# scaomath/galerkin-transformer

Hardware: AMD Instinct MI355X
Metric: training samples/s, Darcy 141x141 Galerkin encoder (fwd+loss+bwd+clip+Adam) (higher is better)
Workload: dtype f32 (operands split into 2 fp16 terms under a running per-row / per-tile power-of-two scale, 3 products on the f16 MFMA pipe, f32 accumulate; fp32-class results: the 1e-5 parity suite passes in this mode; packed-B token GEMMs, convolutions, weight gradients, regression head and the Fourier attention

## Files before the change

galerkin-transformer_amd/csrc/gt_ffn.hip:

```cpp
#include <cstdint>
#include <cstdlib>
#include <algorithm>

#include "gt_common.h"

namespace gt {

typedef __attribute__((address_space(3))) void* ffn_lds_ptr;
typedef const __attribute__((address_space(1))) void* ffn_glb_ptr;

constexpr int FFN_BM = 64, FFN_BK = 16;
constexpr int FFN_STAGE = FFN_BM * FFN_BK * 4;
constexpr int FFN_HSTRIDE = FFN_STAGE + 16;
constexpr int FFN_E0 = 120, FFN_TARGET = 13, FFN_LIMIT = 15;
constexpr int FFN_EP_SW = 36;

__device__ __attribute__((aligned(16))) float ffn_zero[4] = {0.f, 0.f, 0.f, 0.f};

struct FfnP {
    const float* x; const float* res; float* hid; float* out;
    const float* b1; const float* b2;
    const void* Bp1; const void* Bp2;
    int T, d, f;
    int KS1, NT1, KS2, NT2;
    DropDev dh, dout;
    int act;
    uint32_t* bits_out; const uint32_t* bits_in;
    int bwd;
    float e1_scale;
    float* out2; DropDev d2;
};

__device__ __forceinline__ float ffn_alt(int parity) { return (parity & 1) ? -1.f : 1.f; }

__device__ __forceinline__ void ffn_frag(const char* __restrict__ img, int row, int lh, float (&v)[8]) {
    const int s = (row >> 2) & 3;
    const f32x4 a = *reinterpret_cast<const f32x4*>(img + row * 64 + (((2 * lh) ^ s) << 4));
    const f32x4 b = *reinterpret_cast<const f32x4*>(img + row * 64 + (((2 * lh + 1) ^ s) << 4));
    v[0] = a[0]; v[1] = a[1]; v[2] = a[2]; v[3] = a[3];
    v[4] = b[0]; v[5] = b[1]; v[6] = b[2]; v[7] = b[3];
}

template <int NJ>
__device__ __forceinline__ void ffn_tile_stage(const float (&v)[8], int& ea, float sgn, const f16x8 (&bn)[NJ][2],
                                               f32x16 (&acc)[NJ]) {
    float amax = fmaxf(fmaxf(fabsf(v[0]), fabsf(v[1])), fabsf(v[2]));
    amax = fmaxf(fmaxf(amax, fabsf(v[3])), fabsf(v[4]));
    amax = fmaxf(fmaxf(amax, fabsf(v[5])), fabsf(v[6]));
    amax = xor32_max(fmaxf(amax, fabsf(v[7])));
    const int ex = (int)(__float_as_uint(amax) >> 23);
    const bool need = ex + ea - 127 >= FFN_LIMIT;
    if (__any(need)) {
        const int enew = need ? FFN_TARGET + 127 - ex : ea;
        const int dlt = enew - ea;
        const float f = dlt < -126 ? 0.f : pow2_f(dlt);
#pragma unroll
        for (int j = 0; j < NJ; ++j)
#pragma unroll
            for (int e = 0; e < 16; ++e) acc[j][e] *= f;
        ea = enew;
    }
    const float sv = pow2_f(ea) * sgn;
    uint32_t q[4][2];
#pragma unroll
    for (int t = 0; t < 4; ++t) f16_mulsplit_pair(v[2 * t], sv, v[2 * t + 1], sv, q[t][0], q[t][1]);
    f16x8 am[2];
#pragma unroll
    for (int pl = 0; pl < 2; ++pl) am[pl] = __builtin_bit_cast(f16x8, u32x4{q[0][pl], q[1][pl], q[2][pl], q[3][pl]});
#pragma unroll
    for (int s = 1; s >= 0; --s)
#pragma unroll
        for (int pa = 0; pa < 2; ++pa) {
            const int pb = s - pa;
            if (pb < 0 || pb > 1) continue;
#pragma unroll
            for (int j = 0; j < NJ; ++j) acc[j] = __builtin_amdgcn_mfma_f32_32x32x16_f16(bn[j][pb], am[pa], acc[j], 0, 0, 0);
        }
}

__device__ __forceinline__ void ffn_unscale(f32x16& a, int ea, int eb, float sgn) {
    const int et = -(ea + eb), etc = et < -126 ? -126 : (et > 126 ? 126 : et);
    const float sg = pow2_f(etc) * sgn;
#pragma unroll
    for (int e = 0; e < 16; ++e) a[e] *= (e & 1) ? -sg : sg;
    if (et != etc) {
#pragma unroll
        for (int e = 0; e < 16; ++e) a[e] = ldexpf(a[e], et - etc);
    }
}

#define FFN_WAIT_B_(N, bn)                                                                                             \
    asm volatile("s_waitcnt vmcnt(" #N ")" : "+v"(bn[0][0]), "+v"(bn[0][1]), "+v"(bn[1][0]), "+v"(bn[1][1])::"memory")
#define FFN_WAIT_AB_(N, bn)                                                                                            \
    asm volatile("s_waitcnt vmcnt(" #N ")\n\ts_barrier"                                                                \
                 : "+v"(bn[0][0]), "+v"(bn[0][1]), "+v"(bn[1][0]), "+v"(bn[1][1])::"memory")

constexpr int FFN_HST_SW = 68;
constexpr int FFN_PS_TAB = 4 * 64 * FFN_HST_SW * 4;
template <bool PS>
__global__ __launch_bounds__(256, 2) void ffn_fwd16_kernel(const FfnP p) {
    extern __shared__ __attribute__((aligned(16))) char smem[];
    char* const himg = smem;
    const int tid = threadIdx.x, lane = tid & 63, wave = tid >> 6;
    const int lr = lane & 31, lh = lane >> 5;
    int tile;
    {
        const int tiles = gridDim.x, q = tiles >> 3, r = tiles & 7;
        const int x = blockIdx.x & 7, j = blockIdx.x >> 3;
        tile = (x < r ? x * (q + 1) : r * (q + 1) + (x - r) * q) + j;
    }
    const int m0 = tile * FFN_BM;
    const uint32_t voff = lane * 16;

    const int wn_u = __builtin_amdgcn_readfirstlane(wave);
    const char* bbase = reinterpret_cast<const char*>(p.Bp1) + (int64_t)(wn_u * 2) * p.KS1 * 1024;
    const int64_t bplane = (int64_t)p.NT1 * p.KS1 * 1024;
    f16x8 bs0[2][2], bs1[2][2], bs2[2][2];
    auto loadb = [&](int ks, f16x8 (&bn)[2][2]) {
#pragma unroll
        for (int j = 0; j < 2; ++j)
#pragma unroll
            for (int pl = 0; pl < 2; ++pl) {
                const char* sp = bbase + pl * bplane + ((int64_t)j * p.KS1 + ks) * 1024;
                asm volatile("global_load_dwordx4 %0, %1, %2" : "=v"(bn[j][pl]) : "v"(voff), "s"(sp));
            }
    };
    f32x4 b1v[2][4];
#pragma unroll
    for (int j = 0; j < 2; ++j)
#pragma unroll
        for (int g = 0; g < 4; ++g)
            b1v[j][g] = p.b1 ? *reinterpret_cast<const f32x4*>(p.b1 + 64 * wave + 32 * j + 8 * g + 4 * lh) : f32x4{0.f, 0.f, 0.f, 0.f};
    {
        const int row = 16 * wave + (lane >> 2), slot = lane & 3;
        const int g = slot ^ ((row >> 2) & 3);
        const int xr = m0 + row;
        const float* src0 = xr < p.T ? p.x + (int64_t)xr * p.d + 4 * g : ffn_zero;
        const int step = xr < p.T ? FFN_BK : 0;
#pragma unroll
        for (int st = 0; st < 8; ++st)
            __builtin_amdgcn_global_load_lds((ffn_glb_ptr)(src0 + st * step), (ffn_lds_ptr)(himg + st * FFN_HSTRIDE + wave * 1024), 16, 0, 0);
    }
    f32x16 acc[2][2];
#pragma unroll
    for (int i = 0; i < 2; ++i)
#pragma unroll
        for (int j = 0; j < 2; ++j)
#pragma unroll
            for (int e = 0; e < 16; ++e) acc[i][j][e] = 0.f;
    int ea[2] = {FFN_E0, FFN_E0};
    auto stage = [&](int kt, f16x8 (&bn)[2][2]) {
        const char* sa = himg + kt * FFN_HSTRIDE;
#pragma unroll
        for (int i = 0; i < 2; ++i) {
            float v[8];
            ffn_frag(sa, 32 * i + lr, lh, v);
            ffn_tile_stage<2>(v, ea[i], ffn_alt(i), bn, acc[i]);
        }
    };
    loadb(0, bs0); loadb(1, bs1); loadb(2, bs2);
    FFN_WAIT_AB_(8, bs0);
#pragma unroll
    for (int j = 0; j < 2; ++j)
#pragma unroll
        for (int g = 0; g < 4; ++g) asm volatile("" : "+v"(b1v[j][g]));
    stage(0, bs0); loadb(3, bs0);
    FFN_WAIT_B_(8, bs1); stage(1, bs1); loadb(4, bs1);
    FFN_WAIT_B_(8, bs2); stage(2, bs2); loadb(5, bs2);
    FFN_WAIT_B_(8, bs0); stage(3, bs0); loadb(6, bs0);
    FFN_WAIT_B_(8, bs1); stage(4, bs1); loadb(7, bs1);
    FFN_WAIT_B_(8, bs2); stage(5, bs2);
    FFN_WAIT_B_(4, bs0); stage(6, bs0);
    FFN_WAIT_B_(0, bs1); stage(7, bs1);

    const char* bbase2 = reinterpret_cast<const char*>(p.Bp2) + (int64_t)wn_u * p.KS2 * 1024;
    const int64_t bplane2 = (int64_t)p.NT2 * p.KS2 * 1024;
    f16x8 cn0[1][2], cn1[1][2], cn2[1][2], cn3[1][2];
    auto loadb2 = [&](int ks, f16x8 (&bn)[1][2]) {
#pragma unroll
        for (int pl = 0; pl < 2; ++pl) {
            const char* sp = bbase2 + pl * bplane2 + (int64_t)ks * 1024;
            asm volatile("global_load_dwordx4 %0, %1, %2" : "=v"(bn[0][pl]) : "v"(voff), "s"(sp));
        }
    };
    loadb2(0, cn0); loadb2(1, cn1); loadb2(2, cn2); loadb2(3, cn3);
    asm volatile("s_barrier" ::: "memory");

    int er[2] = {0, 0};
    if constexpr (PS) {
        const int* ebp = reinterpret_cast<const int*>(reinterpret_cast<const char*>(p.Bp1) + 2 * bplane) + wn_u * 2;
        const uint32_t key = drop_key_dev(p.dh);
        float* tab = reinterpret_cast<float*>(smem + FFN_PS_TAB);
#pragma unroll
        for (int i = 0; i < 2; ++i) {
            const int row = 32 * i + lr;
            const uint32_t di0 = (uint32_t)((int64_t)(m0 + row) * p.f + 64 * wave + 4 * lh);
            float amax = 0.f;
            const int64_t widx = ((int64_t)(tile * 4 + wave) * 64 + lane) * 2 + i;
            const uint32_t bin = p.bwd ? p.bits_in[widx] : 0u;
            uint32_t bout = 0u;
#pragma unroll
            for (int j = 0; j < 2; ++j) {
                ffn_unscale(acc[i][j], ea[i], ebp[j], ffn_alt(i));
#pragma unroll
                for (int g = 0; g < 4; ++g)
#pragma unroll
                    for (int t = 0; t < 4; ++t) {
                        float y;
                        if (p.bwd) {
                            y = ((bin >> (16 * j + 4 * g + t)) & 1u) ? acc[i][j][4 * g + t] * p.e1_scale : 0.f;
                        } else {
                            y = acc[i][j][4 * g + t] + b1v[j][g][t];
                            if (p.act == GT_ACT_RELU) y = fmaxf(y, 0.f);
                            if (p.dh.thresh) y *= drop_mul(p.dh, key, di0 + 32 * j + 8 * g + t);
                            bout |= (y > 0.f ? 1u : 0u) << (16 * j + 4 * g + t);
                        }
                        acc[i][j][4 * g + t] = y;
                        amax = fmaxf(amax, fabsf(y));
                    }
            }
            if (p.bits_out) p.bits_out[widx] = bout;
            amax = xor32_max(amax);
            if (lh == 0) tab[wave * 64 + row] = amax;
        }
        asm volatile("s_waitcnt lgkmcnt(0)\n\ts_barrier" ::: "memory");
#pragma unroll
        for (int i = 0; i < 2; ++i) {
            const int row = 32 * i + lr;
            const float a = fmaxf(fmaxf(tab[row], tab[64 + row]), fmaxf(tab[128 + row], tab[192 + row]));
            const int ex = (int)(__float_as_uint(a) >> 23);
            er[i] = ex == 0 ? 0 : min(FFN_E0, FFN_TARGET + 127 - ex);
            const float sv = pow2_f(er[i]) * ffn_alt(i);
#pragma unroll
            for (int j = 0; j < 2; ++j)
#pragma unroll
                for (int g = 0; g < 4; ++g) {
                    uint32_t h0, l0, h1, l1;
                    f16_mulsplit_pair(acc[i][j][4 * g], sv, acc[i][j][4 * g + 1], sv, h0, l0);
                    f16_mulsplit_pair(acc[i][j][4 * g + 2], sv, acc[i][j][4 * g + 3], sv, h1, l1);
                    const int st = 4 * wave + 2 * j + (g >> 1);
                    char* dst = smem + (((st * 2 + (g & 1)) * 64 + row) * 16 + lh * 8);
                    *reinterpret_cast<uint2*>(dst) = uint2{h0, h1};
                    *reinterpret_cast<uint2*>(dst + 16 * 64 * 32) = uint2{l0, l1};
                }
        }
    } else {
        const int* ebp = reinterpret_cast<const int*>(reinterpret_cast<const char*>(p.Bp1) + 2 * bplane) + wn_u * 2;
        const uint32_t key = drop_key_dev(p.dh);
#pragma unroll
        for (int i = 0; i < 2; ++i) {
            const int row = 32 * i + lr, swz = (row >> 2) & 3;
            const uint32_t di0 = (uint32_t)((int64_t)(m0 + row) * p.f + 64 * wave + 4 * lh);
#pragma unroll
            for (int j = 0; j < 2; ++j) {
                ffn_unscale(acc[i][j], ea[i], ebp[j], ffn_alt(i));
#pragma unroll
                for (int g = 0; g < 4; ++g) {
                    f32x4 h;
#pragma unroll
                    for (int t = 0; t < 4; ++t) {
                        float y = acc[i][j][4 * g + t] + b1v[j][g][t];
                        if (p.act == GT_ACT_RELU) y = fmaxf(y, 0.f);
                        if (p.dh.thresh) y *= drop_mul(p.dh, key, di0 + 32 * j + 8 * g + t);
                        h[t] = y;
                    }
                    const int st = 4 * wave + 2 * j + (g >> 1), gq = 2 * (g & 1) + lh;
                    *reinterpret_cast<f32x4*>(himg + st * FFN_HSTRIDE + row * 64 + ((gq ^ swz) << 4)) = h;
                }
            }
        }
    }
    asm volatile("s_waitcnt lgkmcnt(0)\n\ts_barrier" ::: "memory");

#define FFN_WAIT_B2_(N, bn) asm volatile("s_waitcnt vmcnt(" #N ")" : "+v"(bn[0][0]), "+v"(bn[0][1])::"memory")
    f32x16 acc2[2][1];
#pragma unroll
    for (int i = 0; i < 2; ++i)
#pragma unroll
        for (int e = 0; e < 16; ++e) acc2[i][0][e] = 0.f;
    int ea2[2] = {FFN_E0, FFN_E0};
    auto stage2 = [&](int kt2, f16x8 (&bn)[1][2]) {
#pragma unroll
        for (int i = 0; i < 2; ++i) {
            if constexpr (PS) {
                const char* fr = smem + (((kt2 * 2 + lh) * 64 + 32 * i + lr) * 16);
                const f16x8 a0 = *reinterpret_cast<const f16x8*>(fr);
                const f16x8 a1 = *reinterpret_cast<const f16x8*>(fr + 16 * 64 * 32);
                acc2[i][0] = __builtin_amdgcn_mfma_f32_32x32x16_f16(bn[0][0], a1, acc2[i][0], 0, 0, 0);
                acc2[i][0] = __builtin_amdgcn_mfma_f32_32x32x16_f16(bn[0][1], a0, acc2[i][0], 0, 0, 0);
                acc2[i][0] = __builtin_amdgcn_mfma_f32_32x32x16_f16(bn[0][0], a0, acc2[i][0], 0, 0, 0);
            } else {
                float v[8];
                ffn_frag(himg + kt2 * FFN_HSTRIDE, 32 * i + lr, lh, v);
                ffn_tile_stage<1>(v, ea2[i], ffn_alt(i), bn, acc2[i]);
            }
        }
    };
    FFN_WAIT_B2_(6, cn0); stage2(0, cn0); loadb2(4, cn0);
    FFN_WAIT_B2_(6, cn1); stage2(1, cn1); loadb2(5, cn1);
    FFN_WAIT_B2_(6, cn2); stage2(2, cn2); loadb2(6, cn2);
    FFN_WAIT_B2_(6, cn3); stage2(3, cn3); loadb2(7, cn3);
    FFN_WAIT_B2_(6, cn0); stage2(4, cn0); loadb2(8, cn0);
    FFN_WAIT_B2_(6, cn1); stage2(5, cn1); loadb2(9, cn1);
    FFN_WAIT_B2_(6, cn2); stage2(6, cn2); loadb2(10, cn2);
    FFN_WAIT_B2_(6, cn3); stage2(7, cn3); loadb2(11, cn3);
    FFN_WAIT_B2_(6, cn0); stage2(8, cn0); loadb2(12, cn0);
    FFN_WAIT_B2_(6, cn1); stage2(9, cn1); loadb2(13, cn1);
    FFN_WAIT_B2_(6, cn2); stage2(10, cn2); loadb2(14, cn2);
    FFN_WAIT_B2_(6, cn3); stage2(11, cn3); loadb2(15, cn3);
    FFN_WAIT_B2_(6, cn0); stage2(12, cn0);
    FFN_WAIT_B2_(4, cn1); stage2(13, cn1);
    FFN_WAIT_B2_(2, cn2); stage2(14, cn2);
    FFN_WAIT_B2_(0, cn3); stage2(15, cn3);
#undef FFN_WAIT_B2_
    {
        const int* ebp2 = reinterpret_cast<const int*>(reinterpret_cast<const char*>(p.Bp2) + 2 * bplane2) + wn_u;
#pragma unroll
        for (int i = 0; i < 2; ++i) ffn_unscale(acc2[i][0], PS ? er[i] : ea2[i], ebp2[0], ffn_alt(i));
    }

    const int c8 = lane & 7, rsub = lane >> 3;
    const int ocol = 32 * wave + 4 * c8;
    f32x4 rs[8];
    if (p.res) {
#pragma unroll
        for (int it = 0; it < 8; ++it) {
            const int m = m0 + 8 * it + rsub;
            rs[it] = m < p.T ? *reinterpret_cast<const f32x4*>(p.res + (int64_t)m * p.d + ocol) : f32x4{0.f, 0.f, 0.f, 0.f};
        }
    }
    const f32x4 b2v = p.b2 ? *reinterpret_cast<const f32x4*>(p.b2 + ocol) : f32x4{0.f, 0.f, 0.f, 0.f};
    if constexpr (PS) {
        asm volatile("s_waitcnt lgkmcnt(0)\n\ts_barrier" ::: "memory");
        float* hs = reinterpret_cast<float*>(smem) + wave * (64 * FFN_HST_SW);
#pragma unroll
        for (int i = 0; i < 2; ++i)
#pragma unroll
            for (int j = 0; j < 2; ++j)
#pragma unroll
                for (int g = 0; g < 4; ++g)
                    *reinterpret_cast<f32x4*>(hs + (32 * i + lr) * FFN_HST_SW + 32 * j + 8 * g + 4 * lh) =
                        f32x4{acc[i][j][4 * g], acc[i][j][4 * g + 1], acc[i][j][4 * g + 2], acc[i][j][4 * g + 3]};
        asm volatile("s_waitcnt lgkmcnt(0)" ::: "memory");
        const int c4 = lane & 15, r4 = lane >> 4;
#pragma unroll 4
        for (int it = 0; it < 16; ++it) {
            const int row = 4 * it + r4;
            const f32x4 h = *reinterpret_cast<const f32x4*>(hs + row * FFN_HST_SW + 4 * c4);
            if (m0 + row < p.T) *reinterpret_cast<f32x4*>(p.hid + (int64_t)(m0 + row) * p.f + 64 * wave + 4 * c4) = h;
        }
        asm volatile("s_waitcnt lgkmcnt(0)" ::: "memory");
    } else {
    {
        const int st = lane >> 2, gq = lane & 3;
#pragma unroll 4
        for (int rr = 0; rr < 16; ++rr) {
            const int row = 16 * wave + rr;
            const f32x4 h = *reinterpret_cast<const f32x4*>(himg + st * FFN_HSTRIDE + row * 64 + ((gq ^ ((row >> 2) & 3)) << 4));
            if (m0 + row < p.T) *reinterpret_cast<f32x4*>(p.hid + (int64_t)(m0 + row) * p.f + 4 * lane) = h;
        }
    }
    asm volatile("s_waitcnt lgkmcnt(0)\n\ts_barrier" ::: "memory");
    }
    {
        float* stg = reinterpret_cast<float*>(smem) + wave * (PS ? 64 * FFN_HST_SW : 64 * FFN_EP_SW);
#pragma unroll
        for (int i = 0; i < 2; ++i)
#pragma unroll
            for (int g = 0; g < 4; ++g)
                *reinterpret_cast<f32x4*>(stg + (32 * i + lr) * FFN_EP_SW + 8 * g + 4 * lh) =
                    f32x4{acc2[i][0][4 * g], acc2[i][0][4 * g + 1], acc2[i][0][4 * g + 2], acc2[i][0][4 * g + 3]};
        asm volatile("s_waitcnt lgkmcnt(0)" ::: "memory");
        const uint32_t key = drop_key_dev(p.dout);
#pragma unroll
        for (int it = 0; it < 8; ++it) {
            const int r = 8 * it + rsub, m = m0 + r;
            f32x4 v = *reinterpret_cast<const f32x4*>(stg + r * FFN_EP_SW + 4 * c8);
            const uint32_t di = (uint32_t)((int64_t)m * p.d + ocol);
#pragma unroll
            for (int t = 0; t < 4; ++t) {
                float y = v[t] + b2v[t];
                if (p.dout.thresh) y *= drop_mul(p.dout, key, di + t);
                v[t] = p.res ? rs[it][t] + y : y;
            }
            if (m < p.T) *reinterpret_cast<f32x4*>(p.out + (int64_t)m * p.d + ocol) = v;
            if (p.out2) {
                const uint32_t key2 = drop_key_dev(p.d2);
                if (p.d2.thresh) {
#pragma unroll
                    for (int t = 0; t < 4; ++t) v[t] *= drop_mul(p.d2, key2, di + t);
                }
                if (m < p.T) *reinterpret_cast<f32x4*>(p.out2 + (int64_t)m * p.d + ocol) = v;
            }
        }
    }
}

}

using namespace gt;

extern "C" int64_t gt_ffn_fwd_ws_bytes(int64_t T, int32_t d, int32_t f) {
    gt_gemm_desc a, b;
    gt_gemm_desc_init(&a); gt_gemm_desc_init(&b);
    a.M = b.M = (int32_t)std::min<int64_t>(T, 1 << 30);
    a.N = f; a.K = d; a.lda = d; a.ldb = d; a.ldc = f; a.precision = GT_PREC_F16X2;
    b.N = d; b.K = f; b.lda = f; b.ldb = f; b.ldc = d; b.precision = GT_PREC_F16X2;
    a.A = a.B = b.A = b.B = reinterpret_cast<const float*>(uintptr_t(16));
    a.C = b.C = reinterpret_cast<float*>(uintptr_t(16));
    const int64_t pa = gt_gemm_packed_b_bytes(&a), pb = gt_gemm_packed_b_bytes(&b);
    return (pa > 0 && pb > 0) ? pa + pb : 0;
}

static int ffn_launch(FfnP& p, const gt_gemm_desc& a, const gt_gemm_desc& b, const void* p1, const void* p2, void* ws,
                      int64_t ws_bytes, void* stream) {
    auto al = [](const void* q) { return (reinterpret_cast<uintptr_t>(q) & 15) == 0; };
    if ((p1 == nullptr) != (p2 == nullptr)) return GT_EINVAL;
    const int64_t pa = gt_gemm_packed_b_bytes(&a), pb = gt_gemm_packed_b_bytes(&b);
    if (pa <= 0 || pb <= 0) return GT_ENOTSUP;
    if (!p1) {
        if (!ws || ws_bytes < pa + pb || !al(ws)) return GT_EWS;
        gt_gemm_desc two[2] = {a, b};
        void* outs[2] = {ws, reinterpret_cast<char*>(ws) + pa};
        if (int rc = gt_gemm_pack_b_many(two, outs, 2, stream)) return rc;
        p1 = outs[0]; p2 = outs[1];
    } else if (!al(p1) || !al(p2)) return GT_EALIGN;
    p.Bp1 = p1; p.Bp2 = p2;
    static const int presplit = [] { const char* e = getenv("GT_FFN_PRESPLIT"); return e ? atoi(e) : 1; }();
    if (!presplit && (p.bwd || p.bits_out)) return GT_ENOTSUP;
    const size_t lds0 = (size_t)16 * FFN_HSTRIDE, lds1 = (size_t)FFN_PS_TAB + 1024;
    const unsigned tiles = (unsigned)(((int64_t)p.T + FFN_BM - 1) / FFN_BM);
    hipStream_t st = (hipStream_t)stream;
    if (presplit) {
        if (int rc = gt_allow_dynamic_lds<ffn_fwd16_kernel<true>>(lds1)) return rc;
        hipLaunchKernelGGL(ffn_fwd16_kernel<true>, dim3(tiles), dim3(256), lds1, st, p);
    } else {
        if (int rc = gt_allow_dynamic_lds<ffn_fwd16_kernel<false>>(lds0)) return rc;
        hipLaunchKernelGGL(ffn_fwd16_kernel<false>, dim3(tiles), dim3(256), lds0, st, p);
    }
    GT_LAUNCH_CHECK();
    return 0;
}

static bool ffn_shape_ok(int64_t T, int32_t d, int32_t f) { return d == 128 && f == 256 && T >= 16384 && T <= (1 << 30); }

extern "C" int64_t gt_ffn_bits_bytes(int64_t T) { return T > 0 ? ((T + FFN_BM - 1) / FFN_BM) * 4 * 64 * 2 * (int64_t)sizeof(uint32_t) : 0; }

extern "C" int gt_ffn_fwd(const float* x, int64_t T, int32_t d, int32_t f, const float* W1, const float* b1,
                          const float* W2, const float* b2, const float* res, const gt_dropout* drop_h,
                          const gt_dropout* drop_o, int32_t act, float* hid, float* out, void* relu_bits,
                          const void* w1_packed, const void* w2_packed, void* ws, int64_t ws_bytes, void* stream) {
    if (!x || !W1 || !W2 || !hid || !out || T <= 0) return GT_EINVAL;
    if (!ffn_shape_ok(T, d, f) || (act != GT_ACT_RELU && act != GT_ACT_NONE)) return GT_ENOTSUP;
    if ((drop_h && drop_h->p > 0.f && !drop_h->seed) || (drop_o && drop_o->p > 0.f && !drop_o->seed)) return GT_EINVAL;
    if ((drop_h && (drop_h->p < 0.f || drop_h->p >= 1.f)) || (drop_o && (drop_o->p < 0.f || drop_o->p >= 1.f))) return GT_EINVAL;
    auto al = [](const void* q) { return (reinterpret_cast<uintptr_t>(q) & 15) == 0; };
    if (!al(x) || !al(W1) || !al(W2) || !al(hid) || !al(out) || !al(res) || !al(b1) || !al(b2) || !al(relu_bits)) return GT_EALIGN;
    gt_gemm_desc a, b;
    gt_gemm_desc_init(&a); gt_gemm_desc_init(&b);
    a.M = b.M = (int32_t)T;
    a.N = f; a.K = d; a.A = x; a.lda = d; a.B = W1; a.ldb = d; a.C = hid; a.ldc = f; a.precision = GT_PREC_F16X2;
    b.N = d; b.K = f; b.A = hid; b.lda = f; b.B = W2; b.ldb = f; b.C = out; b.ldc = d; b.precision = GT_PREC_F16X2;
    FfnP p{x, res, hid, out, b1, b2, nullptr, nullptr, (int)T, d, f,
           d / 16, ((f + 127) / 128) * 4, f / 16, ((d + 127) / 128) * 4, make_drop(drop_h), make_drop(drop_o), act,
           reinterpret_cast<uint32_t*>(relu_bits), nullptr, 0, 1.f, nullptr, make_drop(nullptr)};
    return ffn_launch(p, a, b, w1_packed, w2_packed, ws, ws_bytes, stream);
}

extern "C" int gt_ffn_bwd(const float* gm, int64_t T, int32_t d, int32_t f, const float* W2, const float* W1,
                          const void* relu_bits, float hid_scale, const float* res, float* gh, float* dx, float* dx_masked,
                          const gt_dropout* mask2, const void* w2_packed, const void* w1_packed, void* ws, int64_t ws_bytes,
                          void* stream) {
    if (!gm || !W1 || !W2 || !relu_bits || !gh || !dx || T <= 0) return GT_EINVAL;
    if (!ffn_shape_ok(T, d, f)) return GT_ENOTSUP;
    if (mask2 && (mask2->p < 0.f || mask2->p >= 1.f || (mask2->p > 0.f && !mask2->seed))) return GT_EINVAL;
    auto al = [](const void* q) { return (reinterpret_cast<uintptr_t>(q) & 15) == 0; };
    if (!al(gm) || !al(W1) || !al(W2) || !al(gh) || !al(dx) || !al(res) || !al(dx_masked) || !al(relu_bits)) return GT_EALIGN;
    gt_gemm_desc a, b;
    gt_gemm_desc_init(&a); gt_gemm_desc_init(&b);
    a.M = b.M = (int32_t)T;
    a.N = f; a.K = d; a.A = gm; a.lda = d; a.B = W2; a.ldb = f; a.layout_b = 1; a.C = gh; a.ldc = f; a.precision = GT_PREC_F16X2;
    b.N = d; b.K = f; b.A = gh; b.lda = f; b.B = W1; b.ldb = d; b.layout_b = 1; b.C = dx; b.ldc = d; b.precision = GT_PREC_F16X2;
    FfnP p{gm, res, gh, dx, nullptr, nullptr, nullptr, nullptr, (int)T, d, f,
           d / 16, ((f + 127) / 128) * 4, f / 16, ((d + 127) / 128) * 4, make_drop(nullptr), make_drop(nullptr), GT_ACT_NONE,
           nullptr, reinterpret_cast<const uint32_t*>(relu_bits), 1, hid_scale, dx_masked, make_drop(mask2)};
    return ffn_launch(p, a, b, w2_packed, w1_packed, ws, ws_bytes, stream);
}
```

Before: 6238.

## Make presplit FFN kernel persistent with prefetched next-tile X and residual loads

The presplit FFN forward kernel becomes persistent. The grid is capped at two blocks per CU, and each block loops over a contiguous range of row tiles. The next tile's X rows are prefetched into registers during the epilogue and split into fp16 hi/lo planes in LDS once per tile, instead of being re-split on every MFMA stage. Residual loads, dropout keys and per-column exponent and bias loads are moved earlier or hoisted out of the loop to overlap with compute. This trades higher register pressure and more complex wait counts for less launch/tail overhead and less redundant splitting work.

New measurement: 6214. Within noise of the previous version (-0.4%).

```diff
diff --git a/galerkin-transformer_amd/csrc/gt_ffn.hip b/galerkin-transformer_amd/csrc/gt_ffn.hip
--- a/galerkin-transformer_amd/csrc/gt_ffn.hip
+++ b/galerkin-transformer_amd/csrc/gt_ffn.hip
@@ -97,24 +97,76 @@
 
 constexpr int FFN_HST_SW = 68;
 constexpr int FFN_PS_TAB = 4 * 64 * FFN_HST_SW * 4;
+constexpr int FFN_XPLANE = 8 * 2 * 64 * 16;
 template <bool PS>
 __global__ __launch_bounds__(256, 2) void ffn_fwd16_kernel(const FfnP p) {
     extern __shared__ __attribute__((aligned(16))) char smem[];
     char* const himg = smem;
     const int tid = threadIdx.x, lane = tid & 63, wave = tid >> 6;
     const int lr = lane & 31, lh = lane >> 5;
-    int tile;
+    int tile, tend, tstep;
     {
-        const int tiles = gridDim.x, q = tiles >> 3, r = tiles & 7;
+        const int tiles = (p.T + FFN_BM - 1) / FFN_BM, q = tiles >> 3, r = tiles & 7;
+        const int nb = gridDim.x >> 3, nr = gridDim.x & 7;
         const int x = blockIdx.x & 7, j = blockIdx.x >> 3;
-        tile = (x < r ? x * (q + 1) : r * (q + 1) + (x - r) * q) + j;
-    }
-    const int m0 = tile * FFN_BM;
+        const int t0 = x < r ? x * (q + 1) : r * (q + 1) + (x - r) * q;
+        tile = t0 + j;
+        tend = t0 + (x < r ? q + 1 : q);
+        tstep = nb + (x < nr ? 1 : 0);
+    }
+    if (tile >= tend) return;
     const uint32_t voff = lane * 16;
 
     const int wn_u = __builtin_amdgcn_readfirstlane(wave);
     const char* bbase = reinterpret_cast<const char*>(p.Bp1) + (int64_t)(wn_u * 2) * p.KS1 * 1024;
     const int64_t bplane = (int64_t)p.NT1 * p.KS1 * 1024;
+    const char* bbase2 = reinterpret_cast<const char*>(p.Bp2) + (int64_t)wn_u * p.KS2 * 1024;
+    const int64_t bplane2 = (int64_t)p.NT2 * p.KS2 * 1024;
+    const int xrow = 16 * wave + (lane >> 2), xg = lane & 3;
+    f32x4 xr[8];
+    auto loadx = [&](int t, bool live) {
+        const int r = t * FFN_BM + xrow;
+        const bool in = live && r < p.T;
+        const float* src0 = in ? p.x + (int64_t)r * p.d + 4 * xg : ffn_zero;
+        const int step = in ? FFN_BK : 0;
+#pragma unroll
+        for (int st = 0; st < 8; ++st) asm volatile("global_load_dwordx4 %0, %1, off" : "=v"(xr[st]) : "v"(src0 + st * step));
+    };
+    if constexpr (PS) loadx(tile, true);
+    const uint32_t key_h = drop_key_dev(p.dh);
+    const uint32_t key_o = drop_key_dev(p.dout);
+    const uint32_t key_2 = drop_key_dev(p.d2);
+    const int* ebp = reinterpret_cast<const int*>(reinterpret_cast<const char*>(p.Bp1) + 2 * bplane) + wn_u * 2;
+    const int eb1[2] = {ebp[0], ebp[1]};
+    const int eb2 = (reinterpret_cast<const int*>(reinterpret_cast<const char*>(p.Bp2) + 2 * bplane2))[wn_u];
+    const int c8 = lane & 7, rsub = lane >> 3;
+    const int ocol = 32 * wave + 4 * c8;
+    const f32x4 b2v = p.b2 ? *reinterpret_cast<const f32x4*>(p.b2 + ocol) : f32x4{0.f, 0.f, 0.f, 0.f};
+    if constexpr (PS) {
+        asm volatile("s_waitcnt vmcnt(0)"
+                     : "+v"(xr[0]), "+v"(xr[1]), "+v"(xr[2]), "+v"(xr[3]), "+v"(xr[4]), "+v"(xr[5]), "+v"(xr[6]), "+v"(xr[7])::"memory");
+    }
+
+    for (;;) {
+    const int m0 = tile * FFN_BM;
+    const bool more = tile + tstep < tend;
+    f32x4 rs[8];
+    auto loadres = [&]() {
+#pragma unroll
+        for (int it = 0; it < 8; ++it) {
+            const int m = m0 + 8 * it + rsub;
+            const float* src = (p.res && m < p.T) ? p.res + (int64_t)m * p.d + ocol : ffn_zero;
+            asm volatile("global_load_dwordx4 %0, %1, off" : "=v"(rs[it]) : "v"(src));
+        }
+    };
+    asm volatile("" : "+s"(bbase), "+s"(bbase2));
+    f32x4 b1v[2][4];
+#pragma unroll
+    for (int j = 0; j < 2; ++j)
+#pragma unroll
+        for (int g = 0; g < 4; ++g)
+            b1v[j][g] = p.b1 ? *reinterpret_cast<const f32x4*>(p.b1 + 64 * wave + 32 * j + 8 * g + 4 * lh) : f32x4{0.f, 0.f, 0.f, 0.f};
+
     f16x8 bs0[2][2], bs1[2][2], bs2[2][2];
     auto loadb = [&](int ks, f16x8 (&bn)[2][2]) {
 #pragma unroll
@@ -125,18 +177,12 @@
                 asm volatile("global_load_dwordx4 %0, %1, %2" : "=v"(bn[j][pl]) : "v"(voff), "s"(sp));
             }
     };
-    f32x4 b1v[2][4];
-#pragma unroll
-    for (int j = 0; j < 2; ++j)
-#pragma unroll
-        for (int g = 0; g < 4; ++g)
-            b1v[j][g] = p.b1 ? *reinterpret_cast<const f32x4*>(p.b1 + 64 * wave + 32 * j + 8 * g + 4 * lh) : f32x4{0.f, 0.f, 0.f, 0.f};
-    {
+    if constexpr (!PS) {
         const int row = 16 * wave + (lane >> 2), slot = lane & 3;
         const int g = slot ^ ((row >> 2) & 3);
-        const int xr = m0 + row;
-        const float* src0 = xr < p.T ? p.x + (int64_t)xr * p.d + 4 * g : ffn_zero;
-        const int step = xr < p.T ? FFN_BK : 0;
+        const int xm = m0 + row;
+        const float* src0 = xm < p.T ? p.x + (int64_t)xm * p.d + 4 * g : ffn_zero;
+        const int step = xm < p.T ? FFN_BK : 0;
 #pragma unroll
         for (int st = 0; st < 8; ++st)
             __builtin_amdgcn_global_load_lds((ffn_glb_ptr)(src0 + st * step), (ffn_lds_ptr)(himg + st * FFN_HSTRIDE + wave * 1024), 16, 0, 0);
@@ -149,17 +195,61 @@
 #pragma unroll
             for (int e = 0; e < 16; ++e) acc[i][j][e] = 0.f;
     int ea[2] = {FFN_E0, FFN_E0};
+    uint32_t bin[2] = {0u, 0u};
+    loadb(0, bs0); loadb(1, bs1); loadb(2, bs2);
+    if constexpr (PS) {
+        asm volatile("s_waitcnt lgkmcnt(0)\n\ts_barrier" ::: "memory");
+        {
+            const uint32_t* bsrc = p.bwd ? p.bits_in + ((int64_t)(tile * 4 + wave) * 64 + lane) * 2 : reinterpret_cast<const uint32_t*>(ffn_zero);
+            bin[0] = bsrc[0]; bin[1] = bsrc[1];
+        }
+        float amax = 0.f;
+#pragma unroll
+        for (int st = 0; st < 8; ++st)
+#pragma unroll
+            for (int t = 0; t < 4; ++t) amax = fmaxf(amax, fabsf(xr[st][t]));
+        amax = fmaxf(amax, __shfl_xor(amax, 1));
+        amax = fmaxf(amax, __shfl_xor(amax, 2));
+        const int ex = (int)(__float_as_uint(amax) >> 23);
+        const int ex_row = ex == 0 ? 0 : min(FFN_E0, FFN_TARGET + 127 - ex);
+        const float sv = pow2_f(ex_row) * ffn_alt(xrow >> 5);
+        char* dst = smem + (((xg >> 1) * 64 + xrow) * 16 + (xg & 1) * 8);
+#pragma unroll
+        for (int st = 0; st < 8; ++st) {
+            uint32_t h0, l0, h1, l1;
+            f16_mulsplit_pair(xr[st][0], sv, xr[st][1], sv, h0, l0);
+            f16_mulsplit_pair(xr[st][2], sv, xr[st][3], sv, h1, l1);
+            *reinterpret_cast<uint2*>(dst + st * 2048) = uint2{h0, h1};
+            *reinterpret_cast<uint2*>(dst + st * 2048 + FFN_XPLANE) = uint2{l0, l1};
+        }
+        int* xtab = reinterpret_cast<int*>(smem + FFN_PS_TAB);
+        if (xg == 0) xtab[xrow] = ex_row;
+        asm volatile("s_waitcnt lgkmcnt(0)\n\ts_barrier" ::: "memory");
+#pragma unroll
+        for (int i = 0; i < 2; ++i) ea[i] = xtab[32 * i + lr];
+    }
     auto stage = [&](int kt, f16x8 (&bn)[2][2]) {
-        const char* sa = himg + kt * FFN_HSTRIDE;
 #pragma unroll
         for (int i = 0; i < 2; ++i) {
-            float v[8];
-            ffn_frag(sa, 32 * i + lr, lh, v);
-            ffn_tile_stage<2>(v, ea[i], ffn_alt(i), bn, acc[i]);
+            if constexpr (PS) {
+                const char* fr = smem + (((kt * 2 + lh) * 64 + 32 * i + lr) * 16);
+                const f16x8 a0 = *reinterpret_cast<const f16x8*>(fr);
+                const f16x8 a1 = *reinterpret_cast<const f16x8*>(fr + FFN_XPLANE);
+#pragma unroll
+                for (int j = 0; j < 2; ++j) acc[i][j] = __builtin_amdgcn_mfma_f32_32x32x16_f16(bn[j][1], a0, acc[i][j], 0, 0, 0);
+#pragma unroll
+                for (int j = 0; j < 2; ++j) acc[i][j] = __builtin_amdgcn_mfma_f32_32x32x16_f16(bn[j][0], a1, acc[i][j], 0, 0, 0);
+#pragma unroll
+                for (int j = 0; j < 2; ++j) acc[i][j] = __builtin_amdgcn_mfma_f32_32x32x16_f16(bn[j][0], a0, acc[i][j], 0, 0, 0);
+            } else {
+                float v[8];
+                ffn_frag(himg + kt * FFN_HSTRIDE, 32 * i + lr, lh, v);
+                ffn_tile_stage<2>(v, ea[i], ffn_alt(i), bn, acc[i]);
+            }
         }
     };
-    loadb(0, bs0); loadb(1, bs1); loadb(2, bs2);
-    FFN_WAIT_AB_(8, bs0);
+    if constexpr (PS) FFN_WAIT_B_(8, bs0);
+    else FFN_WAIT_AB_(8, bs0);
 #pragma unroll
     for (int j = 0; j < 2; ++j)
 #pragma unroll
@@ -173,8 +263,7 @@
     FFN_WAIT_B_(4, bs0); stage(6, bs0);
     FFN_WAIT_B_(0, bs1); stage(7, bs1);
 
-    const char* bbase2 = reinterpret_cast<const char*>(p.Bp2) + (int64_t)wn_u * p.KS2 * 1024;
-    const int64_t bplane2 = (int64_t)p.NT2 * p.KS2 * 1024;
+    if constexpr (PS) asm volatile("" : "+v"(bin[0]), "+v"(bin[1]));
     f16x8 cn0[1][2], cn1[1][2], cn2[1][2], cn3[1][2];
     auto loadb2 = [&](int ks, f16x8 (&bn)[1][2]) {
 #pragma unroll
@@ -188,8 +277,6 @@
 
     int er[2] = {0, 0};
     if constexpr (PS) {
-        const int* ebp = reinterpret_cast<const int*>(reinterpret_cast<const char*>(p.Bp1) + 2 * bplane) + wn_u * 2;
-        const uint32_t key = drop_key_dev(p.dh);
         float* tab = reinterpret_cast<float*>(smem + FFN_PS_TAB);
 #pragma unroll
         for (int i = 0; i < 2; ++i) {
@@ -197,22 +284,21 @@
             const uint32_t di0 = (uint32_t)((int64_t)(m0 + row) * p.f + 64 * wave + 4 * lh);
             float amax = 0.f;
             const int64_t widx = ((int64_t)(tile * 4 + wave) * 64 + lane) * 2 + i;
-            const uint32_t bin = p.bwd ? p.bits_in[widx] : 0u;
             uint32_t bout = 0u;
 #pragma unroll
             for (int j = 0; j < 2; ++j) {
-                ffn_unscale(acc[i][j], ea[i], ebp[j], ffn_alt(i));
+                ffn_unscale(acc[i][j], ea[i], eb1[j], ffn_alt(i));
 #pragma unroll
                 for (int g = 0; g < 4; ++g)
 #pragma unroll
                     for (int t = 0; t < 4; ++t) {
                         float y;
                         if (p.bwd) {
-                            y = ((bin >> (16 * j + 4 * g + t)) & 1u) ? acc[i][j][4 * g + t] * p.e1_scale : 0.f;
+                            y = ((bin[i] >> (16 * j + 4 * g + t)) & 1u) ? acc[i][j][4 * g + t] * p.e1_scale : 0.f;
                         } else {
                             y = acc[i][j][4 * g + t] + b1v[j][g][t];
                             if (p.act == GT_ACT_RELU) y = fmaxf(y, 0.f);
-                            if (p.dh.thresh) y *= drop_mul(p.dh, key, di0 + 32 * j + 8 * g + t);
+                            if (p.dh.thresh) y *= drop_mul(p.dh, key_h, di0 + 32 * j + 8 * g + t);
                             bout |= (y > 0.f ? 1u : 0u) << (16 * j + 4 * g + t);
                         }
                         acc[i][j][4 * g + t] = y;
@@ -224,6 +310,7 @@
             if (lh == 0) tab[wave * 64 + row] = amax;
         }
         asm volatile("s_waitcnt lgkmcnt(0)\n\ts_barrier" ::: "memory");
+        loadx(tile + tstep, more);
 #pragma unroll
         for (int i = 0; i < 2; ++i) {
             const int row = 32 * i + lr;
@@ -245,15 +332,13 @@
                 }
         }
     } else {
-        const int* ebp = reinterpret_cast<const int*>(reinterpret_cast<const char*>(p.Bp1) + 2 * bplane) + wn_u * 2;
-        const uint32_t key = drop_key_dev(p.dh);
 #pragma unroll
         for (int i = 0; i < 2; ++i) {
             const int row = 32 * i + lr, swz = (row >> 2) & 3;
             const uint32_t di0 = (uint32_t)((int64_t)(m0 + row) * p.f + 64 * wave + 4 * lh);
 #pragma unroll
             for (int j = 0; j < 2; ++j) {
-                ffn_unscale(acc[i][j], ea[i], ebp[j], ffn_alt(i));
+                ffn_unscale(acc[i][j], ea[i], eb1[j], ffn_alt(i));
 #pragma unroll
                 for (int g = 0; g < 4; ++g) {
                     f32x4 h;
@@ -261,7 +346,7 @@
                     for (int t = 0; t < 4; ++t) {
                         float y = acc[i][j][4 * g + t] + b1v[j][g][t];
                         if (p.act == GT_ACT_RELU) y = fmaxf(y, 0.f);
-                        if (p.dh.thresh) y *= drop_mul(p.dh, key, di0 + 32 * j + 8 * g + t);
+                        if (p.dh.thresh) y *= drop_mul(p.dh, key_h, di0 + 32 * j + 8 * g + t);
                         h[t] = y;
                     }
                     const int st = 4 * wave + 2 * j + (g >> 1), gq = 2 * (g & 1) + lh;
@@ -296,40 +381,36 @@
             }
         }
     };
-    FFN_WAIT_B2_(6, cn0); stage2(0, cn0); loadb2(4, cn0);
-    FFN_WAIT_B2_(6, cn1); stage2(1, cn1); loadb2(5, cn1);
-    FFN_WAIT_B2_(6, cn2); stage2(2, cn2); loadb2(6, cn2);
-    FFN_WAIT_B2_(6, cn3); stage2(3, cn3); loadb2(7, cn3);
+#define FFN_WAIT_B2X_(bn)                                                                                              \
+    do {                                                                                                               \
+        if constexpr (PS) FFN_WAIT_B2_(14, bn);                                                                        \
+        else FFN_WAIT_B2_(6, bn);                                                                                      \
+    } while (0)
+    FFN_WAIT_B2X_(cn0); stage2(0, cn0); loadb2(4, cn0);
+    FFN_WAIT_B2X_(cn1); stage2(1, cn1); loadb2(5, cn1);
+    FFN_WAIT_B2X_(cn2); stage2(2, cn2); loadb2(6, cn2);
+    FFN_WAIT_B2X_(cn3); stage2(3, cn3); loadb2(7, cn3);
+#undef FFN_WAIT_B2X_
     FFN_WAIT_B2_(6, cn0); stage2(4, cn0); loadb2(8, cn0);
+    if constexpr (PS)
+        asm volatile("" : "+v"(xr[0]), "+v"(xr[1]), "+v"(xr[2]), "+v"(xr[3]), "+v"(xr[4]), "+v"(xr[5]), "+v"(xr[6]), "+v"(xr[7]));
     FFN_WAIT_B2_(6, cn1); stage2(5, cn1); loadb2(9, cn1);
     FFN_WAIT_B2_(6, cn2); stage2(6, cn2); loadb2(10, cn2);
     FFN_WAIT_B2_(6, cn3); stage2(7, cn3); loadb2(11, cn3);
-    FFN_WAIT_B2_(6, cn0); stage2(8, cn0); loadb2(12, cn0);
-    FFN_WAIT_B2_(6, cn1); stage2(9, cn1); loadb2(13, cn1);
-    FFN_WAIT_B2_(6, cn2); stage2(10, cn2); loadb2(14, cn2);
-    FFN_WAIT_B2_(6, cn3); stage2(11, cn3); loadb2(15, cn3);
+    loadres();
+    FFN_WAIT_B2_(14, cn0); stage2(8, cn0); loadb2(12, cn0);
+    FFN_WAIT_B2_(14, cn1); stage2(9, cn1); loadb2(13, cn1);
+    FFN_WAIT_B2_(14, cn2); stage2(10, cn2); loadb2(14, cn2);
+    FFN_WAIT_B2_(14, cn3); stage2(11, cn3); loadb2(15, cn3);
     FFN_WAIT_B2_(6, cn0); stage2(12, cn0);
+    asm volatile("" : "+v"(rs[0]), "+v"(rs[1]), "+v"(rs[2]), "+v"(rs[3]), "+v"(rs[4]), "+v"(rs[5]), "+v"(rs[6]), "+v"(rs[7]));
     FFN_WAIT_B2_(4, cn1); stage2(13, cn1);
     FFN_WAIT_B2_(2, cn2); stage2(14, cn2);
     FFN_WAIT_B2_(0, cn3); stage2(15, cn3);
 #undef FFN_WAIT_B2_
-    {
-        const int* ebp2 = reinterpret_cast<const int*>(reinterpret_cast<const char*>(p.Bp2) + 2 * bplane2) + wn_u;
-#pragma unroll
-        for (int i = 0; i < 2; ++i) ffn_unscale(acc2[i][0], PS ? er[i] : ea2[i], ebp2[0], ffn_alt(i));
-    }
-
-    const int c8 = lane & 7, rsub = lane >> 3;
-    const int ocol = 32 * wave + 4 * c8;
-    f32x4 rs[8];
-    if (p.res) {
-#pragma unroll
-        for (int it = 0; it < 8; ++it) {
-            const int m = m0 + 8 * it + rsub;
-            rs[it] = m < p.T ? *reinterpret_cast<const f32x4*>(p.res + (int64_t)m * p.d + ocol) : f32x4{0.f, 0.f, 0.f, 0.f};
-        }
-    }
-    const f32x4 b2v = p.b2 ? *reinterpret_cast<const f32x4*>(p.b2 + ocol) : f32x4{0.f, 0.f, 0.f, 0.f};
+#pragma unroll
+    for (int i = 0; i < 2; ++i) ffn_unscale(acc2[i][0], PS ? er[i] : ea2[i], eb2, ffn_alt(i));
+
     if constexpr (PS) {
         asm volatile("s_waitcnt lgkmcnt(0)\n\ts_barrier" ::: "memory");
         float* hs = reinterpret_cast<float*>(smem) + wave * (64 * FFN_HST_SW);
@@ -371,7 +452,6 @@
                 *reinterpret_cast<f32x4*>(stg + (32 * i + lr) * FFN_EP_SW + 8 * g + 4 * lh) =
                     f32x4{acc2[i][0][4 * g], acc2[i][0][4 * g + 1], acc2[i][0][4 * g + 2], acc2[i][0][4 * g + 3]};
         asm volatile("s_waitcnt lgkmcnt(0)" ::: "memory");
-        const uint32_t key = drop_key_dev(p.dout);
 #pragma unroll
         for (int it = 0; it < 8; ++it) {
             const int r = 8 * it + rsub, m = m0 + r;
@@ -380,19 +460,21 @@
 #pragma unroll
             for (int t = 0; t < 4; ++t) {
                 float y = v[t] + b2v[t];
-                if (p.dout.thresh) y *= drop_mul(p.dout, key, di + t);
+                if (p.dout.thresh) y *= drop_mul(p.dout, key_o, di + t);
                 v[t] = p.res ? rs[it][t] + y : y;
             }
             if (m < p.T) *reinterpret_cast<f32x4*>(p.out + (int64_t)m * p.d + ocol) = v;
             if (p.out2) {
-                const uint32_t key2 = drop_key_dev(p.d2);
                 if (p.d2.thresh) {
 #pragma unroll
-                    for (int t = 0; t < 4; ++t) v[t] *= drop_mul(p.d2, key2, di + t);
+                    for (int t = 0; t < 4; ++t) v[t] *= drop_mul(p.d2, key_2, di + t);
                 }
                 if (m < p.T) *reinterpret_cast<f32x4*>(p.out2 + (int64_t)m * p.d + ocol) = v;
             }
         }
+    }
+    if (!PS || !more) break;
+    tile += tstep;
     }
 }
 
@@ -412,7 +494,19 @@
     return (pa > 0 && pb > 0) ? pa + pb : 0;
 }
 
-static int ffn_launch(FfnP& p, const gt_gemm_desc& a, const gt_gemm_desc& b, const void* p1, const void* p2, void* ws,
+static int ffn_cu_count() {
+    static std::atomic<int> cus[64];
+    int dev = 0;
+    (void)hipGetDevice(&dev);
+    int c = cus[dev & 63].load(std::memory_order_relaxed);
+    if (c <= 0) {
+        if (hipDeviceGetAttribute(&c, hipDeviceAttributeMultiprocessorCount, dev) != hipSuccess || c <= 0) return 0;
+        cus[dev & 63].store(c, std::memory_order_relaxed);
+    }
+    return c;
+}
+
+static int ffn_launch(FfnP& p,const gt_gemm_desc& a, const gt_gemm_desc& b, const void* p1, const void* p2, void* ws,
                       int64_t ws_bytes, void* stream) {
     auto al = [](const void* q) { return (reinterpret_cast<uintptr_t>(q) & 15) == 0; };
     if ((p1 == nullptr) != (p2 == nullptr)) return GT_EINVAL;
@@ -433,7 +527,9 @@
     hipStream_t st = (hipStream_t)stream;
     if (presplit) {
         if (int rc = gt_allow_dynamic_lds<ffn_fwd16_kernel<true>>(lds1)) return rc;
-        hipLaunchKernelGGL(ffn_fwd16_kernel<true>, dim3(tiles), dim3(256), lds1, st, p);
+        const int cus = ffn_cu_count();
+        if (cus <= 0) return GT_ENOTSUP;
+        hipLaunchKernelGGL(ffn_fwd16_kernel<true>, dim3(std::min(tiles, 2u * (unsigned)cus)), dim3(256), lds1, st, p);
     } else {
         if (int rc = gt_allow_dynamic_lds<ffn_fwd16_kernel<false>>(lds0)) return rc;
         hipLaunchKernelGGL(ffn_fwd16_kernel<false>, dim3(tiles), dim3(256), lds0, st, p);
```
